# 0411tony/Yue

Hardware: AMD Instinct MI355X
Metric: BPR triplet-updates/sec at k=128 (S-round semantics, user rows sequential; the reference's exact sequential semantics: secondary.exact) (higher is better)
Workload: dtype f32

## Files before the change

### yue_amd/csrc/bpr_host.hip

```cpp
#include "host_common.hpp"

#include "train_kernels.hpp"
#include "round_kernels.hpp"

using yue_host::fail;
using yue_host::kr_of;
using yue_host::with_kr;
static_assert(yue::kNllSlots == yue_host::kNllSlotsHost && yue::kHeaderSlack == yue_host::kHeaderSlackHost &&
              yue::kMetaStageMax == (uint32_t)yue_host::kMetaStageMaxHost, "host_common.hpp mirrors these");

namespace {

yue::TrainArgs make_args(yue_ctx *c, double lr, double regU, double regI) {
    yue::TrainArgs a{};
    a.P = c->P.p; a.Q = c->Q.p; a.dP = c->dP.p; a.dQ = c->dQ.p;
    a.stage = c->Q.p ? c->Q.p + (size_t)c->n * c->k : nullptr;
    a.ev_u = c->ev_u.p; a.ev_i = c->ev_i.p; a.ev_j = c->ev_j.p;
    a.indptr = c->indptr.p; a.indices = c->indices.p;
    a.nll_slots = c->scal.p;
    a.m = c->m; a.n = c->n; a.k = c->k;
    a.lr = lr;
    a.ru = (float)(lr * regU);
    a.ri = (float)(lr * regI);
    a.neg_lo = 0; a.neg_range = (int32_t)c->n;
// ... 19 lines not shown
template <class F>
bool with_round_instance(int kr, int tpw, F &&f) {
    return with_round_instance(kr, tpw, f, std::make_index_sequence<sizeof kRoundInstances / sizeof kRoundInstances[0]>{});
}

int tpw_of(const yue_ctx *c, bool meta) { return c->opt_round_tpw ? c->opt_round_tpw : default_round_tpw(kr_of(c->k), meta); }

constexpr int64_t kMetaRangeMax = 37 * 1024;
constexpr int64_t kMetaRangesMax = 12;
constexpr int64_t kRoundGenerationsMax = 6;
constexpr double kRoundEventsPerItemRow = 4.0;

bool meta_bucketed(const yue_ctx *c) { return c->n > kMetaRangeMax * kMetaRangesMax || c->opt_round_bucket; }
bool meta_path_fits(const yue_ctx *c) { return c->opt_round_meta && c->n <= ((int64_t)yue::kBucketRangesMax << yue::kBucketShift); }

int default_round_events(yue_ctx *c, double n_rows, int64_t *out) {
    const bool fold = yue_host::fold_path(c);
    const int tpw = tpw_of(c, fold);
    int per_cu = 0, cus = 0;
    hipError_t e = hipSuccess;
    if (!with_round_instance(kr_of(c->k), tpw, [&](auto kr, auto t) {
            e = fold ? hipOccupancyMaxActiveBlocksPerMultiprocessor(&per_cu, yue::k_round_m<kr(), t()>, 256, 0)
                     : hipOccupancyMaxActiveBlocksPerMultiprocessor(&per_cu, yue::k_round<kr(), t()>, 256, 0);
        }))
        return fail(YUE_ERR_ARG, "unsupported (k, TPW) combination");
    HIPCHK(e);
    per_cu = std::min(per_cu, fold ? 7 : 6);
    HIPCHK(hipDeviceGetAttribute(&cus, hipDeviceAttributeMultiprocessorCount, c->device));
    const double slots = (double)per_cu * (double)cus;
    int64_t w = (int64_t)(slots * 4.0 * tpw);
    w -= w % 1024;
    w = std::max<int64_t>(w, 1024);
    if (fold) {
        int64_t sets = std::min<int64_t>(kRoundGenerationsMax, std::max<int64_t>(1, (int64_t)(kRoundEventsPerItemRow * n_rows / (double)w)));
        if (2.0 * (double)(w * sets) < 2.0 * n_rows) sets = std::min<int64_t>(sets, 4);
        w *= sets;
    }
    *out = w;
    return YUE_OK;
}

int launch_round(yue_ctx *c, const yue::TrainArgs &a_in, int64_t e0, int64_t e1, int64_t n0, int64_t n1,
                 int parity, int apply_p) {
    unsigned long long *cnt[2] = {c->cnt0.p, c->cnt1.p};
    uint32_t *cntp[2] = {c->cntp0.p, c->cntp1.p};
    yue::RoundArgs ra{};
    ra.e_begin = e0; ra.e_end = e1; ra.n_begin = n0; ra.n_end = n1;
    ra.cnt_cur = cnt[parity]; ra.cnt_next = cnt[parity ^ 1]; ra.cntp_cur = cntp[parity]; ra.cntp_next = cntp[parity ^ 1];
    uint32_t *tab[2] = {c->tab0.p, c->tab1.p};
    ra.tab_cur = tab[parity]; ra.tab_next = tab[parity ^ 1]; ra.staged = c->staged ? 1 : 0;
    ra.apply_p = apply_p;
    const int tpw = tpw_of(c, false);
    const int64_t waves = (std::max(e1 - e0, n1 - n0) + tpw - 1) / tpw;
    const int64_t blocks = (waves + 3) / 4;
    if (blocks == 0) return YUE_OK;
    const dim3 grid((unsigned)blocks), block(256);
#ifdef YUE_STAMPS
    yue::TrainArgs a = a_in;
    a.stamps = nullptr;
    if (e1 > e0 && c->update_launches++ == c->stamp_launch) {
        HIPCHK(c->stamps.resize((size_t)waves * 8));
        HIPCHK(hipMemsetAsync(c->stamps.p, 0, (size_t)waves * 64, c->stream));
        a.stamps = c->stamps.p;
        c->stamp_waves = (e1 - e0 + tpw - 1) / tpw;
    }
#else
    const yue::TrainArgs &a = a_in;
#endif
    if (!with_round_instance(kr_of(c->k), tpw, [&](auto kr, auto t) {
            hipLaunchKernelGGL((yue::k_round<kr(), t()>), grid, block, 0, c->stream, a, ra, a.ev_u, a.ev_i, a.ev_j);
        }))
        return fail(YUE_ERR_ARG, "unsupported (k, TPW) combination");
    return YUE_OK;
}

int launch_round_meta(yue_ctx *c, const yue::TrainArgs &a, const std::vector<int64_t> &bounds) {
    const int64_t R = (int64_t)bounds.size() - 1;
    const int64_t E = bounds.back();
    HIPCHK(c->meta_i.resize((size_t)E + yue::kHeaderSlack)); HIPCHK(c->meta_j.resize((size_t)E + yue::kHeaderSlack));
    HIPCHK(c->round_rows.resize((size_t)R)); HIPCHK(c->d_bounds.resize((size_t)R + 1));
    if (c->h_bounds != bounds) {
        HIPCHK(hipStreamSynchronize(c->stream));
        c->h_bounds = bounds;
        HIPCHK(hipMemcpyAsync(c->d_bounds.p, c->h_bounds.data(), (size_t)(R + 1) * sizeof(int64_t), hipMemcpyHostToDevice, c->stream));
    }
    HIPCHK(hipMemsetAsync(c->round_rows.p, 0, (size_t)R * sizeof(unsigned long long), c->stream));
    HIPCHK(c->fold.resize((size_t)(E + 4 * R + 8)));
    yue::MetaArgs ma{};
    ma.ev_i = a.ev_i; ma.ev_j = a.ev_j; ma.bounds = c->d_bounds.p; ma.R = R; ma.n = (int32_t)c->n;
    const bool bucketed = meta_bucketed(c);
    if (bucketed) {
        ma.range = 1 << yue::kBucketShift;
        ma.G = (int32_t)((c->n + ma.range - 1) >> yue::kBucketShift);
        HIPCHK(c->bk_touch.resize((size_t)(2 * E + 2))); HIPCHK(c->bk_ptr.resize((size_t)R * (ma.G + 1)));
        yue::BucketArgs ba{};
        ba.ev_i = a.ev_i; ba.ev_j = a.ev_j; ba.bounds = c->d_bounds.p; ba.R = R; ba.G = ma.G;
        ba.bk_touch = c->bk_touch.p; ba.bk_ptr = c->bk_ptr.p; ba.meta_i = c->meta_i.p; ba.meta_j = c->meta_j.p;
        int cus0 = 0;
        HIPCHK(hipDeviceGetAttribute(&cus0, hipDeviceAttributeMultiprocessorCount, c->device));
        hipLaunchKernelGGL(yue::k_round_bucket, dim3((unsigned)std::min<int64_t>(R, 2 * cus0)), dim3(1024), 0, c->stream, ba);
        ma.bk_touch = c->bk_touch.p; ma.bk_ptr = c->bk_ptr.p;
    } else {
        ma.G = (int32_t)((c->n + kMetaRangeMax - 1) / kMetaRangeMax);
        ma.range = (int32_t)((c->n + ma.G - 1) / ma.G);
    }
    ma.chunk = (ma.range + 1023) / 1024; ma.chunk |= 1;
    int64_t widest = 0;
    for (int64_t r = 0; r < R; ++r) widest = std::max(widest, bounds[(size_t)r + 1] - bounds[(size_t)r]);
    const double mean_touches = 2.0 * (double)widest / (double)std::max<int64_t>(1, c->n);
    const uint32_t stage_auto = (uint32_t)std::min<double>((double)yue::kMetaStageMax, std::max<double>((double)yue::kMetaStageDefault,
                                                         std::ceil(mean_touches * (kr_of(c->k) == 1 ? 4.0 : 2.0))));
    ma.stage_max = !c->staged ? 1u : c->opt_round_stage >= 2 ? (uint32_t)c->opt_round_stage : stage_auto;
    c->last_stage_max = (int)ma.stage_max;
    ma.meta_i = c->meta_i.p; ma.meta_j = c->meta_j.p; ma.round_rows = c->round_rows.p; ma.fold = c->fold.p;
    const size_t lds = (size_t)ma.range * sizeof(uint32_t);
    const void *kfn = bucketed ? (const void *)yue::k_round_meta<true> : (const void *)yue::k_round_meta<false>;
    HIPCHK(hipFuncSetAttribute(kfn, hipFuncAttributeMaxDynamicSharedMemorySize, (int)lds));
    int per_cu = 0, cus = 0;
    if (bucketed) { HIPCHK(hipOccupancyMaxActiveBlocksPerMultiprocessor(&per_cu, yue::k_round_meta<true>, 1024, lds)); }
    else { HIPCHK(hipOccupancyMaxActiveBlocksPerMultiprocessor(&per_cu, yue::k_round_meta<false>, 1024, lds)); }
    HIPCHK(hipDeviceGetAttribute(&cus, hipDeviceAttributeMultiprocessorCount, c->device));
    const int64_t grid = std::max<int64_t>(8, std::min<int64_t>((R * ma.G + 7) / 8 * 8, (int64_t)std::max(per_cu, 1) * cus / 8 * 8));
    if (bucketed) hipLaunchKernelGGL(yue::k_round_meta<true>, dim3((unsigned)grid), dim3(1024), lds, c->stream, ma);
    else
        hipLaunchKernelGGL(yue::k_round_meta<false>, dim3((unsigned)grid), dim3(1024), lds, c->stream, ma);
    HIPCHK(hipGetLastError());
    return YUE_OK;
}

void launch_round_fold(yue_ctx *c, const yue::TrainArgs &a, int64_t e0, int64_t e1, int64_t round_index) {
    yue::FoldArgs f{};
    f.fold = c->fold.p + yue::fold_base(e0, round_index); f.round_rows = c->round_rows.p + round_index; f.Q = a.Q; f.dQ = a.dQ; f.stage = a.stage; f.k = c->k; f.capacity = (uint32_t)((e1 - e0) & ~(int64_t)3);
    const dim3 fgrid((unsigned)std::min<int64_t>(c->opt_fold_blocks, std::max<int64_t>(1, (e1 - e0 + 15) / 16))), block(256);
    with_kr(c->k, [&](auto kr) { hipLaunchKernelGGL(yue::k_round_fold<kr()>, fgrid, block, 0, c->stream, f); });
}

int launch_round_m(yue_ctx *c, const yue::TrainArgs &a_in, int64_t e0, int64_t e1, int64_t round_index) {
    yue::RoundMArgs ra{};
    ra.e_begin = e0; ra.e_end = e1; ra.staged = c->staged ? 1 : 0;
    const int tpw = tpw_of(c, true);
    const int64_t waves = (e1 - e0 + tpw - 1) / tpw;
    const int64_t blocks = (waves + 3) / 4;
    if (blocks == 0) return YUE_OK;
    const dim3 grid((unsigned)blocks), block(256);
#ifdef YUE_STAMPS
    yue::TrainArgs a = a_in;
    a.stamps = nullptr;
    if (c->update_launches++ == c->stamp_launch) {
        HIPCHK(c->stamps.resize((size_t)waves * 8));
        HIPCHK(hipMemsetAsync(c->stamps.p, 0, (size_t)waves * 64, c->stream));
        a.stamps = c->stamps.p;
        c->stamp_waves = waves;
    }
#else
    const yue::TrainArgs &a = a_in;
#endif
    const uint32_t *mi = c->meta_i.p, *mj = c->meta_j.p;
    if (c->bigq) {
        bool is_default = false;
        with_round_instance(kr_of(c->k), tpw, [&](auto kr, auto t) {
            if constexpr (t() == default_round_tpw(kr(), true)) {
                hipLaunchKernelGGL((yue::k_round_m<kr(), t(), true>), grid, block, 0, c->stream, a, ra, a.ev_u, a.ev_i, a.ev_j, mi, mj);
                is_default = true;
            }
        });
        if (!is_default) return fail(YUE_ERR_ARG, "item matrices of 2 GiB and more: only the default events-per-wave setting (round_tpw = 0)");
    } else if (!with_round_instance(kr_of(c->k), tpw, [&](auto kr, auto t) {
                   hipLaunchKernelGGL((yue::k_round_m<kr(), t()>), grid, block, 0, c->stream, a, ra, a.ev_u, a.ev_i, a.ev_j, mi, mj);
               }))
        return fail(YUE_ERR_ARG, "unsupported (k, TPW) combination");
    launch_round_fold(c, a, e0, e1, round_index);
    return YUE_OK;
}

int launch_round_u(yue_ctx *c, const yue::TrainArgs &a, int64_t u0, int64_t u1, int64_t e0, int64_t e1, int64_t round_index) {
    yue::RoundUArgs ra{};
    ra.u_begin = u0; ra.u_end = u1; ra.ev_ptr = c->d_ev_ptr.p; ra.e_begin = e0; ra.e_end = e1; ra.staged = c->staged ? 1 : 0; ra.margins = c->margins.p;
    ra.psq_slots = c->psq_in_rounds ? c->psq_slots.p : nullptr;
    const int64_t blocks = (u1 - u0 + 3) / 4;
    if (blocks == 0) return YUE_OK;
    const dim3 grid((unsigned)blocks), block(256);
    const uint32_t *mi = c->meta_i.p, *mj = c->meta_j.p;
    with_kr(c->k, [&](auto kr) {
        if (c->opt_round_fast) hipLaunchKernelGGL((yue::k_round_u<kr(), true>), grid, block, 0, c->stream, a, ra, a.ev_i, a.ev_j, mi, mj);
        else hipLaunchKernelGGL((yue::k_round_u<kr(), false>), grid, block, 0, c->stream, a, ra, a.ev_i, a.ev_j, mi, mj);
    });
    launch_round_fold(c, a, e0, e1, round_index);
    return YUE_OK;
}

template <typename F>
int run_rounds(yue_ctx *c, yue::TrainArgs a, const std::vector<int64_t> &bounds, int apply_p, F after_round, bool meta = false, const std::vector<int64_t> *user_blocks = nullptr) {
    const int64_t R = (int64_t)bounds.size() - 1;
    int64_t widest = 0;
    for (int64_t r = 0; r < R; ++r) widest = std::max(widest, bounds[(size_t)r + 1] - bounds[(size_t)r]);
    if (widest >= (1ll << 24)) meta = false;
    const bool fits31 = (c->n + 2 * widest) * (int64_t)c->k * 4 < (1ll << 31);
    c->bigq = meta && !fits31;
    if (!meta && (int64_t)c->n * c->k * 4 >= (1ll << 31))
        return fail(YUE_ERR_ARG, "item matrices of 2 GiB and more per GPU are supported by yue_bpr_epoch's default path only (not by explicit rounds / round_meta = 0 / rounds of 2^24 events and more)");
    c->staged = c->opt_round_stage && widest > 0 && (fits31 || c->bigq);
    if (c->staged) {
        const size_t need = (size_t)(c->n + 2 * widest) * (size_t)c->k;
        if (c->Q.n < need) {
            DevBuf<float> bigger;
            HIPCHK(bigger.resize(need));
// ... 450 lines not shown
```

### yue_amd/csrc/core_host.hip

```cpp
#include "host_common.hpp"

namespace yue_host {
thread_local std::string g_err;
int fail(int code, const std::string &msg) { g_err = msg; return code; }
}
using yue_host::fail;
void yue_comm_release(yue_ctx *c);

extern "C" {

const char *yue_last_error(void) { return yue_host::g_err.c_str(); }
int yue_version(void) { return 1; }

int yue_ctx_create(int device, yue_ctx **out) {
    if (!out) return fail(YUE_ERR_ARG, "yue_ctx_create: out is NULL");
    int ndev = 0;
    HIPCHK(hipGetDeviceCount(&ndev));
    if (ndev <= 0) return fail(YUE_ERR_HIP, "no HIP device visible: libyue_hip needs an MI355X (no CPU fallback exists)");
    if (device < 0 || device >= ndev) return fail(YUE_ERR_ARG, "device ordinal out of range");
    HIPCHK(hipSetDevice(device));
    yue_ctx *c = new yue_ctx();
    c->device = device;
    const auto init = [c]() -> int {
        HIPCHK(hipStreamCreateWithFlags(&c->stream, hipStreamNonBlocking));
// ... 15 lines not shown

int yue_ctx_destroy(yue_ctx *c) {
    if (!c) return YUE_OK;
    (void)hipSetDevice(c->device);
    if (c->stream) (void)hipStreamSynchronize(c->stream);
    if (c->comm_stream) (void)hipStreamSynchronize(c->comm_stream);
    yue_comm_release(c);
    if (c->comm_stream) (void)hipStreamDestroy(c->comm_stream);
    if (c->stream) (void)hipStreamDestroy(c->stream);
    delete c;
    return YUE_OK;
}

int yue_sync(yue_ctx *c) {
    if (!c) return fail(YUE_ERR_ARG, "null context");
    HIPCHK(hipSetDevice(c->device));
    HIPCHK(hipStreamSynchronize(c->stream));
    return YUE_OK;
}

int yue_set_factors(yue_ctx *c, const float *P, int64_t m, const float *Q, int64_t n, int k) {
    if (!c || !P || !Q) return fail(YUE_ERR_ARG, "yue_set_factors: null argument");
    if (m <= 0 || n <= 0 || k <= 0 || k > 256) return fail(YUE_ERR_ARG, "yue_set_factors: need m,n > 0 and 1 <= k <= 256");
    if (n >= (1ll << 31) || m >= (1ll << 31)) return fail(YUE_ERR_ARG, "yue_set_factors: ids must fit int32");
    HIPCHK(hipSetDevice(c->device));
    if (c->have_inter && (m != c->m || n != c->n || k != c->k)) c->have_inter = false;
    if (k != c->k) c->opt_round_tpw = 0;
    c->m = m; c->n = n; c->k = k;
    HIPCHK(c->P.resize(m * k)); HIPCHK(c->Q.resize(n * k));
    HIPCHK(c->dP.resize(m * k)); HIPCHK(c->dQ.resize(n * k));
    HIPCHK(c->cnt0.resize(n)); HIPCHK(c->cnt1.resize(n)); HIPCHK(c->cntp0.resize(m)); HIPCHK(c->cntp1.resize(m));
    HIPCHK(hipMemcpyAsync(c->P.p, P, m * k * sizeof(float), hipMemcpyHostToDevice, c->stream));
    HIPCHK(hipMemcpyAsync(c->Q.p, Q, n * k * sizeof(float), hipMemcpyHostToDevice, c->stream));
    HIPCHK(hipMemsetAsync(c->dP.p, 0, m * k * sizeof(float), c->stream));
    HIPCHK(hipMemsetAsync(c->dQ.p, 0, n * k * sizeof(float), c->stream));
    HIPCHK(hipMemsetAsync(c->cntp0.p, 0, m * sizeof(uint32_t), c->stream));
    HIPCHK(hipMemsetAsync(c->cntp1.p, 0, m * sizeof(uint32_t), c->stream));
    HIPCHK(hipMemsetAsync(c->cnt0.p, 0, n * sizeof(unsigned long long), c->stream));
    HIPCHK(hipMemsetAsync(c->cnt1.p, 0, n * sizeof(unsigned long long), c->stream));
    HIPCHK(hipStreamSynchronize(c->stream));
    c->have_factors = true;
    return YUE_OK;
}

int yue_get_factors(yue_ctx *c, float *P, float *Q) {
    if (!c || !c->have_factors) return fail(YUE_ERR_ARG, "yue_get_factors: no factors uploaded");
    HIPCHK(hipSetDevice(c->device));
    if (P) HIPCHK(hipMemcpyAsync(P, c->P.p, c->m * c->k * sizeof(float), hipMemcpyDeviceToHost, c->stream));
    if (Q) HIPCHK(hipMemcpyAsync(Q, c->Q.p, c->n * c->k * sizeof(float), hipMemcpyDeviceToHost, c->stream));
    HIPCHK(hipStreamSynchronize(c->stream));
    return YUE_OK;
}

int yue_set_interactions(yue_ctx *c, const int64_t *indptr, const int32_t *indices, const int64_t *ev_ptr, const int32_t *ev_i) {
    if (!c || !indptr || !indices || !ev_ptr || !ev_i) return fail(YUE_ERR_ARG, "yue_set_interactions: null argument");
    if (!c->have_factors) return fail(YUE_ERR_ARG, "yue_set_interactions: call yue_set_factors first (m, n)");
    HIPCHK(hipSetDevice(c->device));
    const int64_t m = c->m, n = c->n;
    int rc = check_rows("yue_set_interactions: interaction", indptr, m, indices, n, yue_host::kNoTotal, Order::ascending);
    if (!rc) rc = check_rows("yue_set_interactions: event", ev_ptr, m, ev_i, n, yue_host::kNoTotal, Order::any);
    if (rc) return rc;
    for (int64_t u = 0; u < m; ++u)
        if (indptr[u + 1] - indptr[u] >= n) return fail(YUE_ERR_ARG, "yue_set_interactions: a user listened to every item (the reference's sampler would never return, BPR.py:47)");
    const int64_t nnz = indptr[m], E = ev_ptr[m];
    {
        int64_t prev = -1, max_gap = 0;
        for (int64_t u = 0; u < m; ++u) if (ev_ptr[u + 1] > ev_ptr[u]) { if (prev >= 0) max_gap = std::max(max_gap, u - prev); prev = u; }
        if (max_gap * c->k * 4 >= (1ll << 31)) return fail(YUE_ERR_ARG, "yue_set_interactions: more than 2 GiB of user-factor rows between two consecutive users with events");
    }
    std::vector<int32_t> evu((size_t)E);
    for (int64_t u = 0; u < m; ++u)
        for (int64_t e = ev_ptr[u]; e < ev_ptr[u + 1]; ++e) evu[(size_t)e] = (int32_t)u;
    c->E = E; c->nnz = nnz;
    c->h_ev_ptr.assign(ev_ptr, ev_ptr + m + 1);
    c->all_users_have_events = true;
    for (int64_t u = 0; u < m; ++u) if (ev_ptr[u + 1] <= ev_ptr[u]) { c->all_users_have_events = false; break; }
    c->d_ev_ptr_valid = false;
    HIPCHK(c->indptr.resize(m + 1)); HIPCHK(c->indices.resize(std::max<int64_t>(nnz, 1)));
    HIPCHK(c->ev_u.resize((size_t)E + yue_host::kHeaderSlackHost)); HIPCHK(c->ev_i.resize((size_t)E + yue_host::kHeaderSlackHost)); HIPCHK(c->ev_j.resize((size_t)E + yue_host::kHeaderSlackHost));
    HIPCHK(hipMemcpyAsync(c->indptr.p, indptr, (m + 1) * sizeof(int64_t), hipMemcpyHostToDevice, c->stream));
    HIPCHK(hipMemcpyAsync(c->indices.p, indices, nnz * sizeof(int32_t), hipMemcpyHostToDevice, c->stream));
    HIPCHK(hipMemcpyAsync(c->ev_u.p, evu.data(), E * sizeof(int32_t), hipMemcpyHostToDevice, c->stream));
    HIPCHK(hipMemcpyAsync(c->ev_i.p, ev_i, E * sizeof(int32_t), hipMemcpyHostToDevice, c->stream));
    HIPCHK(hipStreamSynchronize(c->stream));
    c->have_inter = true;
    return YUE_OK;
}


}
```

### yue_amd/csrc/host_common.hpp

```cpp
#pragma once
#include "../../include/yue_hip.h"
#include "input_checks.hpp"

#include <hip/hip_runtime.h>

#include <algorithm>
#include <cmath>
#include <cstdio>
#include <cstdlib>
#include <cstring>
#include <memory>
#include <string>
#include <type_traits>
#include <utility>
#include <vector>

struct ncclComm;
struct yue_wrmf;
struct yue_knn;
struct yue_expo;
struct yue_cof;
struct yue_cnet;
struct yue_s2v;
struct yue_lgcn;
// ... 49 lines not shown
    return YUE_OK;
}

struct Event {
    hipEvent_t e = nullptr;
    Event() = default;
    Event(const Event &) = delete;
    Event &operator=(const Event &) = delete;
    Event(Event &&o) noexcept : e(o.e) { o.e = nullptr; }
    Event &operator=(Event &&o) noexcept { std::swap(e, o.e); return *this; }
    ~Event() { if (e) (void)hipEventDestroy(e); }
    hipError_t create(unsigned flags = hipEventDefault) { return e ? hipSuccess : hipEventCreateWithFlags(&e, flags); }
    hipError_t record(hipStream_t s) {
        const hipError_t rc = create();
        return rc != hipSuccess ? rc : hipEventRecord(e, s);
    }
    operator hipEvent_t() const { return e; }
};

inline hipError_t elapsed(hipEvent_t from, hipEvent_t to, double *ms) {
    float f = 0.0f;
    const hipError_t rc = hipEventElapsedTime(&f, from, to);
    if (rc == hipSuccess) *ms = (double)f;
    return rc;
}
inline int64_t ns_of(double ms) { return (int64_t)(1e6 * ms); }
inline hipError_t elapsed(hipEvent_t from, hipEvent_t to, int64_t *ns) {
    double ms = 0.0;
    const hipError_t rc = elapsed(from, to, &ms);
    if (rc == hipSuccess) *ns = ns_of(ms);
    return rc;
}

constexpr int kNllSlotsHost = 1024;
constexpr int kHeaderSlackHost = 16;
constexpr int kMetaStageMaxHost = 64;
constexpr int kWrmfStageHost = 32;
constexpr int kKnnRangeHost = 4096, kKnnMaxKHost = 256, kKnnGatherHost = 2048;
constexpr int kCofRangeHost = 8192;

template <class T>
using StatePtr = std::unique_ptr<T, void (*)(T *)>;

inline int kr_of(int k) { return k <= 64 ? 1 : k <= 128 ? 2 : 4; }

template <class F>
auto with_kr(int k, F &&f) {
    switch (kr_of(k)) {
        case 1: return f(std::integral_constant<int, 1>{});
        case 2: return f(std::integral_constant<int, 2>{});
        default: return f(std::integral_constant<int, 4>{});
    }
}

}

using yue_host::DevBuf;
using yue_host::Event;
using yue_host::Order;
using yue_host::check_ids;
using yue_host::check_rows;
using yue_host::check_transpose;

struct yue_ctx {
    int device = 0;
    hipStream_t stream = nullptr;
    int64_t m = 0, n = 0, E = 0, nnz = 0;
    int k = 0;
    bool have_factors = false, have_inter = false;
    DevBuf<float> P, Q, dP, dQ;
    DevBuf<float> margins;
    DevBuf<double> psq_slots;
    DevBuf<unsigned long long> cnt0, cnt1;
    DevBuf<uint32_t> cntp0, cntp1;
    DevBuf<uint32_t> tab0, tab1;
    bool staged = false;
    bool bigq = false;
    DevBuf<uint32_t> meta_i, meta_j;
    DevBuf<unsigned long long> round_rows;
    DevBuf<uint2> fold, bk_touch;
    DevBuf<uint32_t> bk_ptr;
    DevBuf<int64_t> d_bounds;
    std::vector<int64_t> h_bounds;
#ifdef YUE_STAMPS
    DevBuf<unsigned long long> stamps;
    int64_t stamp_launch = -1, update_launches = 0, stamp_waves = 0;
#endif
    DevBuf<int32_t> ev_u, ev_i, ev_j, indices;
    DevBuf<int64_t> indptr;
    DevBuf<int32_t> xu, xi, xj, xk;
    DevBuf<double> x_loss;
    DevBuf<float> aU_m, aU_v, aV_m, aV_v;
    int64_t adam_m = 0, adam_n = 0; int adam_k = 0;
    DevBuf<double> scal;
    std::vector<int64_t> h_ev_ptr;
    bool all_users_have_events = false;
    bool psq_in_rounds = false;
    DevBuf<int32_t> s_users, s_ids, s_mask_idx, s_flags;
    DevBuf<int32_t> s_few, s_few_ids;
    DevBuf<float> s_few_scores;
    int64_t scan_few_users = 0;
    DevBuf<int64_t> s_mask_ptr;
    DevBuf<float> s_scores, s_row, s_norms;
    double scan_ms = 0.0;
    int64_t scan_events = 0, scan_rescored = 0, scan_tiles_done = 0, scan_tiles_total = 0;
    DevBuf<unsigned long long> s_work;
    DevBuf<unsigned short> s_qb;
    DevBuf<uint32_t> s_masks;
    int opt_scan_two_phase = 1;
    int64_t opt_scan_streams_min_users = 262144;
    int opt_scan_slabs = 4;
    int opt_scan_streams = 2;
    int opt_scan_filter_ub = 3;
    int opt_scan_growth = 0;
    int scan_chunks = 0;
    int scan_used_bf16 = 0;
    int opt_scan_f32 = 0;
    int opt_scan_batch = 0;
    int opt_round_tpw = 0;
    int opt_topn_true = 0;
    int scan_settle = 0;
    int last_stage_max = 0;
    int opt_round_stage = 1;
    int opt_round_bucket = 0;
    int opt_fold_blocks = 1536;
    int opt_round_user_seq = 1;
    int opt_round_fast = 1;
    int last_round_user_seq = 0;
    int opt_comm_group_mb = 8;
    int opt_round_cus_reserved = 0;
    int64_t comm_compute_waits = 0;
    int opt_round_meta = 1;
    int timing_stride = 0;
    std::vector<std::pair<Event, Event>> ev_pool;
    std::vector<int64_t> ev_triplets, ev_launches;
    size_t ev_used = 0;
    DevBuf<double> fP, fBi, f_coef, f_x, f_hist, f_scores, f_out_sc;
    DevBuf<float> fQ;
    DevBuf<int64_t> f_ptr;
    DevBuf<int32_t> f_items, f_negs, f_ids, f_flags;
    DevBuf<int64_t> f_uq_ptr, f_neg_ptr;
    DevBuf<int32_t> f_uq_items, f_loc_i, f_loc_j;
    DevBuf<float> f_wq, f_dQ;
    DevBuf<double> f_wp, f_wb, f_dP, f_dB;
    DevBuf<unsigned> f_cnt;
    int64_t fn = 0;
    int fk = 0;
    int opt_fism_inplace = 1;
    int opt_fism_lds = 1;
    int64_t fism_form = 0;
    DevBuf<uint32_t> ch_key, ch_val, ch_key2, ch_val2, ch_seg, ch_ord_i, ch_ord_j, ch_head, ch_incl, ch_ord_u, ch_rkey, ch_rval;
    DevBuf<int64_t> ch_run_ptr, d_ev_ptr;
    DevBuf<int32_t> ch_run_u;
    DevBuf<unsigned char> ch_tmp;
    DevBuf<unsigned> ch_Qv, ch_Pv;
    DevBuf<unsigned long long> ch_ctl;
    DevBuf<unsigned long long> ch_stats;
    bool d_ev_ptr_valid = false;
    int opt_epoch_exact = 0;
    int opt_replay_levels = 0;
    int opt_chain_split = -1;
    int opt_chain_ring = 0;
    int opt_chain_xcd = 0;
    int opt_chain_fast = 0;
    int opt_chain_waves = 0;
    int64_t opt_chain_spin = 0;
// ... 90 lines not shown
```

### yue_amd/csrc/options_host.hip

```cpp
#include "host_common.hpp"

#include <limits>

using yue_host::fail;

namespace {

struct Option {
    const char *name;
    int64_t (*get)(yue_ctx *);
    void (*put)(yue_ctx *, int64_t);
    int (*set)(const Option &, yue_ctx *, int64_t);
    int64_t lo, hi;
    const char *refusal;
    std::vector<int64_t> also;
};
#define YUE_AT(member) [](yue_ctx *c) -> int64_t { return c->member; }, [](yue_ctx *c, int64_t v) { c->member = (decltype(c->member))v; }
#define YUE_FROM(reader) [](yue_ctx *c) -> int64_t { return yue_host::reader; }

int set_flag(const Option &o, yue_ctx *c, int64_t value) { o.put(c, value != 0); return YUE_OK; }

int set_ranged(const Option &o, yue_ctx *c, int64_t value) {
    if ((value < o.lo || value > o.hi) && std::find(o.also.begin(), o.also.end(), value) == o.also.end())
        return fail(YUE_ERR_ARG, std::string("yue_set_option: ") + o.name + " " + o.refusal);
    o.put(c, value);
    return YUE_OK;
}

int64_t round_path(yue_ctx *c) { return yue_host::fold_path(c) ? 1 : 0; }

int set_round_cus_reserved(const Option &, yue_ctx *c, int64_t value) {
    int cus = 0;
    HIPCHK(hipSetDevice(c->device));
    HIPCHK(hipDeviceGetAttribute(&cus, hipDeviceAttributeMultiprocessorCount, c->device));
    if (value < 0 || value >= cus) return fail(YUE_ERR_ARG, "yue_set_option: round_cus_reserved must be 0 .. CUs - 1");
    HIPCHK(hipStreamSynchronize(c->stream));
    hipStream_t fresh = nullptr;
    if (value == 0) HIPCHK(hipStreamCreateWithFlags(&fresh, hipStreamNonBlocking));
    else {
        std::vector<uint32_t> mask((size_t)(cus + 31) / 32, 0u);
        for (int cu = 0; cu < cus - (int)value; ++cu) mask[(size_t)cu / 32] |= 1u << (cu % 32);
        HIPCHK(hipExtStreamCreateWithCUMask(&fresh, (uint32_t)mask.size(), mask.data()));
    }
    (void)hipStreamDestroy(c->stream);
    c->stream = fresh;
    c->opt_round_cus_reserved = (int)value;
    return YUE_OK;
}

int set_round_tpw(const Option &, yue_ctx *c, int64_t value) {
    if (value != 0 && value != 2 && value != 4 && value != 8 && value != 16) return fail(YUE_ERR_ARG, "yue_set_option: round_tpw must be 0, 2, 4, 8 or 16");
    if (value == 8 && yue_host::kr_of(c->k) == 4) return fail(YUE_ERR_ARG, "yue_set_option: round_tpw 8 needs k <= 128");
    if (value == 16 && yue_host::kr_of(c->k) != 1) return fail(YUE_ERR_ARG, "yue_set_option: round_tpw 16 needs k <= 64");
    c->opt_round_tpw = (int)value;
    return YUE_OK;
}

#ifdef YUE_STAMPS
int set_stamp_launch(const Option &, yue_ctx *c, int64_t value) { c->stamp_launch = value; c->update_launches = 0; return YUE_OK; }
#endif

constexpr int64_t kNoEnd = std::numeric_limits<int64_t>::max();

const Option kOptions[] = {
    {"scan_f32", YUE_AT(opt_scan_f32), set_flag},
    {"scan_batch", YUE_AT(opt_scan_batch), set_ranged, 0, 1, "must be 0 or 1"},
    {"scan_two_phase", YUE_AT(opt_scan_two_phase), set_flag},
    {"scan_growth", YUE_AT(opt_scan_growth), set_ranged, 2, 64, "must be 0 (automatic) or 2..64", {0}},
    {"scan_filter_ub", YUE_AT(opt_scan_filter_ub), set_ranged, 1, 3, "must be 1, 2 or 3"},
    {"scan_streams", YUE_AT(opt_scan_streams), set_ranged, 1, 2, "must be 1 or 2"},
    {"scan_slabs", YUE_AT(opt_scan_slabs), set_ranged, 2, 64, "must be 2..64"},
    {"scan_streams_min_users", YUE_AT(opt_scan_streams_min_users), set_ranged, 1024, kNoEnd, "must be at least 1024"},
    {"scan_last_chunks", YUE_AT(scan_chunks)},
    {"scan_last_few_users", YUE_AT(scan_few_users)},
    {"scan_last_settle", YUE_AT(scan_settle)},
    {"topn_true", YUE_AT(opt_topn_true), set_flag},
    {"fism_lds", YUE_AT(opt_fism_lds), set_flag},
    {"fism_inplace", YUE_AT(opt_fism_inplace), set_flag},
    {"fism_last_form", YUE_AT(fism_form)},
    {"round_stage", YUE_AT(opt_round_stage), set_ranged, 0, yue_host::kMetaStageMaxHost, "must be 0, 1 or 2..64"},
    {"round_last_stage_max", YUE_AT(last_stage_max)},
    {"round_meta", YUE_AT(opt_round_meta), set_flag},
    {"comm_group_mb", YUE_AT(opt_comm_group_mb), set_ranged, 1, 4096, "must be 1..4096"},
    {"round_cus_reserved", YUE_AT(opt_round_cus_reserved), set_round_cus_reserved},
    {"comm_last_compute_waits", YUE_AT(comm_compute_waits)},
    {"round_user_seq", YUE_AT(opt_round_user_seq), set_flag},
    {"round_fast", YUE_AT(opt_round_fast), set_flag},
    {"round_last_user_seq", YUE_AT(last_round_user_seq)},
    {"round_bucket", YUE_AT(opt_round_bucket), set_flag},
    {"fold_blocks", YUE_AT(opt_fold_blocks), set_ranged, 1, 65536, "out of range"},
    {"round_tpw", YUE_AT(opt_round_tpw), set_round_tpw},
    {"round_path", round_path},
#ifdef YUE_STAMPS
    {"debug_stamp_launch", nullptr, nullptr, set_stamp_launch},
#endif
    {"epoch_exact", YUE_AT(opt_epoch_exact), set_flag},
    {"replay_levels", YUE_AT(opt_replay_levels), set_flag},
    {"chain_waves", YUE_AT(opt_chain_waves), set_ranged, 0, 8, "must be 0..8"},
    {"chain_split", YUE_AT(opt_chain_split), set_ranged, -1, 1, "must be -1, 0 or 1"},
    {"chain_fast", YUE_AT(opt_chain_fast), set_flag},
    {"chain_xcd", YUE_AT(opt_chain_xcd), set_flag},
    {"chain_ring", YUE_AT(opt_chain_ring), set_ranged, 0, 0, "must be 0, 8 or 16", {8, 16}},
    {"chain_spin", YUE_AT(opt_chain_spin), set_ranged, 0, 0x7fffffff, "out of range"},
    {"chain_last_us", YUE_AT(chain_kernel_us)},
    {"chain_last_runs", YUE_AT(chain_runs)},
    {"chain_last_waves", YUE_AT(chain_waves)},
    {"replay_last_levels", YUE_AT(replay_levels)},
    {"lgcn_hub", YUE_AT(opt_lgcn_hub), set_ranged, 1, 0x7fffffff, "must be 1 .. 2^31 - 1"},
    {"lgcn_last_hubs", YUE_AT(lgcn_hubs)},
    {"lgcn_last_parts", YUE_AT(lgcn_parts)},
    {"lgcn_last_forward_ns", YUE_AT(lgcn_ns[0])},
    {"lgcn_last_batch_ns", YUE_AT(lgcn_ns[1])},
    {"lgcn_last_backward_ns", YUE_AT(lgcn_ns[2])},
    {"lgcn_last_adam_ns", YUE_AT(lgcn_ns[3])},
    {"ngcf_hub", YUE_AT(opt_ngcf_hub), set_ranged, 1, 0x7fffffff, "must be 1 .. 2^31 - 1"},
    {"ngcf_last_hubs", YUE_AT(ngcf_hubs)},
    {"ngcf_last_parts", YUE_AT(ngcf_parts)},
    {"ngcf_last_gather_ns", YUE_AT(ngcf_ns[0])},
    {"ngcf_last_dense_ns", YUE_AT(ngcf_ns[1])},
    {"ngcf_last_batch_ns", YUE_AT(ngcf_ns[2])},
    {"ngcf_last_backward_ns", YUE_AT(ngcf_ns[3])},
    {"ngcf_last_wgrad_ns", YUE_AT(ngcf_ns[4])},
    {"ngcf_last_adam_ns", YUE_AT(ngcf_ns[5])},
    {"cdae_hub", YUE_AT(opt_cdae_hub), set_ranged, 1, 0x7fffffff, "must be 1 .. 2^31 - 1"},
    {"cdae_last_hubs", YUE_AT(cdae_hubs)},
    {"cdae_last_parts", YUE_AT(cdae_parts)},
    {"cdae_last_saturated", YUE_AT(cdae_saturated)},
    {"apr_last_longest_row", YUE_AT(apr_longest)},
    {"wrmf_long_pairs", YUE_AT(opt_wrmf_long_pairs), set_ranged, yue_host::kWrmfStageHost, kNoEnd, "must be >= 32"},
    {"wrmf_last_ns", YUE_AT(wrmf_ns[0])},
    {"wrmf_last_long_ns", YUE_AT(wrmf_ns[1])},
    {"wrmf_long_rows_user", YUE_FROM(wrmf_long_rows(c, 0))},
    {"wrmf_long_rows_item", YUE_FROM(wrmf_long_rows(c, 1))},
    {"knn_range", YUE_AT(opt_knn_range), set_ranged, 64, yue_host::kKnnRangeHost, "must be 64..4096"},
    {"knn_gather", YUE_AT(opt_knn_gather), set_ranged, yue_host::kKnnMaxKHost, yue_host::kKnnGatherHost, "must be 256..2048"},
    {"knn_last_ns", YUE_AT(knn_ns)},
    {"knn_last_chunked_users", YUE_AT(knn_chunked_users)},
    {"ipf_slots", YUE_AT(opt_ipf_slots), set_ranged, 1, 4096, "must be 1..4096"},
    {"ipf_last_ns", YUE_AT(ipf_ns)},
    {"expo_gram_mb", YUE_AT(opt_expo_gram_mb), set_ranged, 1, 65536, "must be in [1, 65536]"},
    {"expo_last_ns", YUE_AT(expo_ns[0])},
    {"expo_last_gram_ns", YUE_AT(expo_ns[1])},
    {"expo_last_batches", YUE_AT(expo_batches)},
    {"cof_cooccur_mb", YUE_AT(opt_cof_cooccur_mb), set_ranged, 1, 65536, "must be in [1, 65536]"},
    {"cof_level_timing", YUE_AT(opt_cof_level_timing), set_ranged, 0, 1, "must be 0 or 1"},
    {"cof_pass_items", YUE_AT(opt_cof_pass_items), set_ranged, 64, yue_host::kCofRangeHost, "must be in [64, 8192]"},
    {"cof_last_ns", YUE_AT(cof_ns[0])},
    {"cof_last_small_ns", YUE_AT(cof_ns[1])},
    {"cof_levels", YUE_FROM(cof_levels(c))},
    {"cof_cooccur_nnz", YUE_FROM(cof_cooccur_nnz(c))},
    {"cnet_last_ns", YUE_AT(cnet_ns)},
    {"s2v_schedule", YUE_AT(opt_s2v_schedule), set_ranged, 0, 1, "must be 0 (one wave walks all steps) or 1 (levels)"},
    {"s2v_levels_steps", YUE_FROM(s2v_levels(c, 0))},
    {"s2v_levels_pairs", YUE_FROM(s2v_levels(c, 1))},
    {"s2v_last_ns", YUE_AT(s2v_ns)},
};
#undef YUE_AT
#undef YUE_FROM

const Option *find_option(const std::string &key) {
    for (const Option &o : kOptions) if (key == o.name) return &o;
    return nullptr;
}

}

extern "C" {

int yue_get_option(yue_ctx *c, const char *name, int64_t *value) {
    if (!c || !name || !value) return fail(YUE_ERR_ARG, "yue_get_option: null argument");
    const std::string key(name);
    const Option *o = find_option(key);
    if (o && o->get) { *value = o->get(c); return YUE_OK; }
    return fail(YUE_ERR_ARG, "yue_get_option: unknown option " + key);
}
// ... 11 lines not shown
```

### yue_amd/csrc/round_kernels.hpp

```cpp
#pragma once
#include "train_kernels.hpp"

#ifdef YUE_ABL_NO_HOT
#define YUE_M_HOT(val, rs, vo, so) asm volatile("" :: "v"(val))
#else
#define YUE_M_HOT(val, rs, vo, so) YUE_BATOMIC(val, rs, vo, so)
#endif
#ifdef YUE_ABL_NO_DP
#define YUE_M_DP(val, rs, vo, so) asm volatile("" :: "v"(val))
#else
#define YUE_M_DP(val, rs, vo, so) YUE_BATOMIC(val, rs, vo, so)
#endif

#define YUE_BLOAD_NT(rs, vo, so) __builtin_bit_cast(float, __builtin_amdgcn_raw_buffer_load_b32((rs), (vo), (so), 2))
#if defined(YUE_EXP_LOAD_CACHED)
#define YUE_M_LOAD_J(rs, vo, so) YUE_BLOAD(rs, vo, so)
#define YUE_M_LOAD_I(rs, vo, so) YUE_BLOAD(rs, vo, so)
#elif defined(YUE_EXP_LOAD_NT)
#define YUE_M_LOAD_J(rs, vo, so) YUE_BLOAD_NT(rs, vo, so)
#define YUE_M_LOAD_I(rs, vo, so) YUE_BLOAD_NT(rs, vo, so)
#else
#define YUE_M_LOAD_J(rs, vo, so) YUE_BLOAD_NT(rs, vo, so)
#define YUE_M_LOAD_I(rs, vo, so) YUE_BLOAD(rs, vo, so)
#endif

#define YUE_FOLD_LD(p) __builtin_nontemporal_load(p)
#define YUE_FOLD_LDROW(p) (*(p))

namespace yue {

constexpr uint32_t kMetaStageMax = 64u;
constexpr uint32_t kMetaStageDefault = 4u;
constexpr uint32_t kMetaUnique = 1u, kMetaStaged = 2u, kMetaHot = 3u;
constexpr uint32_t kMetaFirst = 1u << 31;
constexpr int kMetaUnroll = 8;
__host__ __device__ inline uint32_t meta_kind(uint32_t w) { return w & 3u; }
__host__ __device__ inline uint32_t meta_slot(uint32_t w) { return (w >> 2) & 0x1fffffffu; }
__host__ __device__ inline bool meta_first(uint32_t w) { return (w & kMetaFirst) != 0u; }
__host__ __device__ inline uint32_t fold_count(uint32_t w) { return w >> 25; }
__host__ __device__ inline uint32_t fold_block(uint32_t w) { return w & 0x1ffffffu; }
constexpr uint32_t kLdsStaged = 1u << 31, kLdsTicket = 1u << 25;
static_assert(kMetaStageMax <= 64u, "tickets of a block must fit bits 25..30 of the LDS word");
__device__ inline uint32_t meta_of_staged(uint32_t lds) {
    const uint32_t ticket = (lds >> 25) & 63u;
    return kMetaStaged | (((lds & 0x1ffffffu) + ticket) << 2) | (ticket == 0u ? kMetaFirst : 0u);
}

struct MetaArgs {
    const int32_t *ev_i, *ev_j;
    const int64_t *bounds;
    int64_t R;
    int32_t n;
    int32_t range;
    int32_t G;
    int32_t chunk;
    uint32_t stage_max;
    uint32_t *meta_i, *meta_j;
    unsigned long long *round_rows;
    uint2 *fold;
    const uint2 *bk_touch;
    const uint32_t *bk_ptr;
};

__host__ __device__ inline int64_t fold_base(int64_t e0, int64_t r) { return (e0 + 4 * r + 3) & ~(int64_t)3; }

template <bool BUCKETED>
__global__ void __launch_bounds__(1024) k_round_meta(MetaArgs a) {
    extern __shared__ uint32_t slots[];
    __shared__ unsigned long long wsum[16];
    __shared__ unsigned long long range_base;
    const int tid = threadIdx.x, lane = tid & 63, wv = tid >> 6;
    const int64_t xcd = blockIdx.x & 7, local = blockIdx.x >> 3, per_xcd = gridDim.x >> 3;
    const int64_t rounds_here = (a.R - xcd + 7) >> 3;
    for (int64_t sq = local; sq < rounds_here * a.G; sq += per_xcd) {
        const int64_t r = (sq / a.G) * 8 + xcd;
        const int32_t g = (int32_t)(sq % a.G);
        const int32_t lo = g * a.range;
        const int32_t width = min(a.range, a.n - lo);
        const int64_t e0 = a.bounds[r], e1 = a.bounds[r + 1];
        for (int s = tid; s < a.range; s += 1024) slots[s] = 0u;
        __syncthreads();
        const uint2 *mine_t = nullptr;
        uint32_t mine_n = 0u;
        if (BUCKETED) {
            const uint32_t *bp = a.bk_ptr + r * (a.G + 1) + g;
            mine_t = a.bk_touch + 2 * e0 + bp[0];
            mine_n = bp[1] - bp[0];
        }
        if (BUCKETED) {
            for (uint32_t t = tid; t < mine_n; t += 1024) atomicAdd(&slots[mine_t[t].x - (uint32_t)lo], 1u);
        } else {
        for (int64_t eb = e0 + tid; eb < e1; eb += 1024 * kMetaUnroll) {
            int32_t vi[kMetaUnroll], vj[kMetaUnroll];
#pragma unroll
            for (int q = 0; q < kMetaUnroll; ++q) {
                const int64_t e = eb + 1024 * q;
                vj[q] = e < e1 ? a.ev_j[e] : -1; vi[q] = e < e1 ? a.ev_i[e] : 0;
            }
#pragma unroll
            for (int q = 0; q < kMetaUnroll; ++q)
                if (vj[q] >= 0) {
                    const uint32_t si = (uint32_t)(vi[q] - lo), sj = (uint32_t)(vj[q] - lo);
                    if (si < (uint32_t)width) atomicAdd(&slots[si], 1u);
                    if (sj < (uint32_t)width) atomicAdd(&slots[sj], 1u);
                }
        }
        }
        __syncthreads();
        const int s0 = tid * a.chunk;
        unsigned long long mine = 0ull;
        for (int q = 0; q < a.chunk; ++q) {
            const int s = s0 + q;
            if (s < width) { const uint32_t c = slots[s]; if (c >= 2u) mine += (1ull << 32) + (c <= a.stage_max ? c : 0u); }
        }
        unsigned long long incl = mine;
#pragma unroll
        for (int off = 1; off < 64; off <<= 1) { const unsigned long long up = __shfl_up(incl, off); if (lane >= off) incl += up; }
        if (lane == 63) wsum[wv] = incl;
        __syncthreads();
        if (tid == 0) {
            unsigned long long total = 0ull;
            for (int q = 0; q < 16; ++q) total += wsum[q];
            range_base = total ? atomicAdd(a.round_rows + r, total) : 0ull;
        }
        __syncthreads();
        unsigned long long run = range_base + incl - mine;
        for (int q = 0; q < wv; ++q) run += wsum[q];
        uint2 *fold = a.fold + fold_base(e0, r);
        for (int q = 0; q < a.chunk; ++q) {
            const int s = s0 + q;
            if (s < width) {
                const uint32_t c = slots[s];
                if (c >= 2u) {
                    const bool st = c <= a.stage_max;
                    slots[s] = st ? (kLdsStaged | ((uint32_t)run & 0x1ffffffu)) : kMetaHot;
                    fold[run >> 32] = make_uint2((uint32_t)(lo + s), st ? ((c << 25) | ((uint32_t)run & 0x1ffffffu)) : 0u);
                    run += (1ull << 32) + (st ? c : 0u);
                }
            }
        }
        __syncthreads();
        if (BUCKETED) {
            for (uint32_t t = tid; t < mine_n; t += 1024) {
                const uint2 tc = mine_t[t];
                const uint32_t sl = tc.x - (uint32_t)lo;
                const uint32_t wd = slots[sl];
                const uint32_t mw = (wd & kLdsStaged) ? meta_of_staged(atomicAdd(&slots[sl], kLdsTicket)) : wd;
                ((tc.y & 1u) ? a.meta_j : a.meta_i)[e0 + (tc.y >> 1)] = mw;
            }
        } else
        for (int64_t eb = e0 + tid; eb < e1; eb += 1024 * kMetaUnroll) {
            int32_t vi[kMetaUnroll], vj[kMetaUnroll];
#pragma unroll
            for (int q = 0; q < kMetaUnroll; ++q) {
                const int64_t e = eb + 1024 * q;
                vj[q] = e < e1 ? a.ev_j[e] : -1; vi[q] = e < e1 ? a.ev_i[e] : 0;
            }
#pragma unroll
            for (int q = 0; q < kMetaUnroll; ++q) {
                const int64_t e = eb + 1024 * q;
                if (vj[q] >= 0) {
                    const uint32_t si = (uint32_t)(vi[q] - lo), sj = (uint32_t)(vj[q] - lo);
                    if (si < (uint32_t)width) {
                        const uint32_t wd = slots[si];
                        a.meta_i[e] = (wd & kLdsStaged) ? meta_of_staged(atomicAdd(&slots[si], kLdsTicket)) : wd;
                    }
                    if (sj < (uint32_t)width) {
                        const uint32_t wd = slots[sj];
                        a.meta_j[e] = (wd & kLdsStaged) ? meta_of_staged(atomicAdd(&slots[sj], kLdsTicket)) : wd;
                    }
                } else if (g == 0 && e < e1) {
                    a.meta_i[e] = 0u; a.meta_j[e] = 0u;
                }
            }
        }
        __syncthreads();
    }
}

constexpr int kBucketShift = 15;
constexpr int kBucketRangesMax = 256;
struct BucketArgs {
    const int32_t *ev_i, *ev_j;
    const int64_t *bounds;
    int64_t R;
    int32_t G;
    uint2 *bk_touch;
    uint32_t *bk_ptr;
    uint32_t *meta_i, *meta_j;
};

__global__ void __launch_bounds__(1024) k_round_bucket(BucketArgs a) {
    __shared__ uint32_t cnt[kBucketRangesMax], off[kBucketRangesMax + 1];
    const int tid = threadIdx.x;
    for (int64_t r = blockIdx.x; r < a.R; r += gridDim.x) {
        const int64_t e0 = a.bounds[r], e1 = a.bounds[r + 1];
        for (int g = tid; g < a.G; g += 1024) cnt[g] = 0u;
        __syncthreads();
        for (int64_t eb = e0 + tid; eb < e1; eb += 1024 * kMetaUnroll) {
            int32_t vi[kMetaUnroll], vj[kMetaUnroll];
#pragma unroll
            for (int q = 0; q < kMetaUnroll; ++q) {
                const int64_t e = eb + 1024 * q;
                vj[q] = e < e1 ? a.ev_j[e] : 0; vi[q] = e < e1 ? a.ev_i[e] : -1;
            }
#pragma unroll
            for (int q = 0; q < kMetaUnroll; ++q) {
                if (vi[q] < 0) continue;
                if (vj[q] >= 0) { atomicAdd(&cnt[vi[q] >> kBucketShift], 1u); atomicAdd(&cnt[vj[q] >> kBucketShift], 1u); }
                else { a.meta_i[eb + 1024 * q] = 0u; a.meta_j[eb + 1024 * q] = 0u; }
            }
        }
        __syncthreads();
        if (tid == 0) {
            uint32_t run = 0u;
            for (int g = 0; g < a.G; ++g) { off[g] = run; run += cnt[g]; cnt[g] = 0u; }
            off[a.G] = run;
        }
        __syncthreads();
        for (int g = tid; g <= a.G; g += 1024) a.bk_ptr[r * (a.G + 1) + g] = off[g];
        uint2 *dst = a.bk_touch + 2 * e0;
        for (int64_t eb = e0 + tid; eb < e1; eb += 1024 * kMetaUnroll) {
            int32_t vi[kMetaUnroll], vj[kMetaUnroll];
#pragma unroll
            for (int q = 0; q < kMetaUnroll; ++q) {
                const int64_t e = eb + 1024 * q;
                vj[q] = e < e1 ? a.ev_j[e] : -1; vi[q] = e < e1 ? a.ev_i[e] : 0;
            }
#pragma unroll
            for (int q = 0; q < kMetaUnroll; ++q)
                if (vj[q] >= 0) {
                    const uint32_t code = 2u * (uint32_t)(eb + 1024 * q - e0);
                    const int gi = vi[q] >> kBucketShift, gj = vj[q] >> kBucketShift;
                    dst[off[gi] + atomicAdd(&cnt[gi], 1u)] = make_uint2((uint32_t)vi[q], code);
                    dst[off[gj] + atomicAdd(&cnt[gj], 1u)] = make_uint2((uint32_t)vj[q], code | 1u);
                }
        }
        __syncthreads();
    }
}


struct RoundMArgs {
    int64_t e_begin, e_end;
    int staged;
};

template <int KR, int TPW, bool BIGQ = false>
__global__ void __launch_bounds__(256) __attribute__((amdgpu_num_sgpr(96))) k_round_m(TrainArgs a, RoundMArgs ra, const int32_t *__restrict__ evu,
                                                 const int32_t *__restrict__ evi, const int32_t *__restrict__ evj,
                                                 const uint32_t *__restrict__ mti, const uint32_t *__restrict__ mtj) {
    const int lane = threadIdx.x & 63;
    const int64_t wave = (int64_t)blockIdx.x * 4 + __builtin_amdgcn_readfirstlane((int)(threadIdx.x >> 6));
    const int64_t base = ra.e_begin + wave * TPW;
    if (base >= ra.e_end) return;
    YUE_STAMP(0, "");

// ... 399 lines not shown
```

Baseline: 1.785 billion.

## Cache per-round positive-item touch counts across epochs in meta pre-pass

Adds a one-time kernel that counts positive-item touches per round and range and packs them as saturating 8-bit counts. The meta kernel then seeds its LDS histogram from this cache and only atomically adds negative-item touches. This drops half the per-epoch ev_i reads and LDS atomics. The cost is extra device memory, a cold-path correction for invalid events, a saturation bias encoding and cache invalidation logic.

Result: no change. 1.787 billion (median of 6 runs) (+0.1%).

```diff
diff --git a/yue_amd/csrc/bpr_host.hip b/yue_amd/csrc/bpr_host.hip
--- a/yue_amd/csrc/bpr_host.hip
+++ b/yue_amd/csrc/bpr_host.hip
@@ -125,6 +125,7 @@
     if (c->h_bounds != bounds) {
         HIPCHK(hipStreamSynchronize(c->stream));
         c->h_bounds = bounds;
+        c->pos_cnt_valid = false;
         HIPCHK(hipMemcpyAsync(c->d_bounds.p, c->h_bounds.data(), (size_t)(R + 1) * sizeof(int64_t), hipMemcpyHostToDevice, c->stream));
     }
     HIPCHK(hipMemsetAsync(c->round_rows.p, 0, (size_t)R * sizeof(unsigned long long), c->stream));
@@ -156,15 +157,31 @@
     ma.stage_max = !c->staged ? 1u : c->opt_round_stage >= 2 ? (uint32_t)c->opt_round_stage : stage_auto;
     c->last_stage_max = (int)ma.stage_max;
     ma.meta_i = c->meta_i.p; ma.meta_j = c->meta_j.p; ma.round_rows = c->round_rows.p; ma.fold = c->fold.p;
-    const size_t lds = (size_t)ma.range * sizeof(uint32_t);
-    const void *kfn = bucketed ? (const void *)yue::k_round_meta<true> : (const void *)yue::k_round_meta<false>;
+    ma.pos_words = (ma.range + 3) / 4;
+    const int64_t pos_total = R * ma.G * (int64_t)ma.pos_words;
+    const bool static_pos = !bucketed && c->opt_meta_static_pos && a.ev_i == c->ev_i.p && pos_total * 4 <= (c->opt_meta_static_cap_mb << 20);
+    c->last_meta_static = static_pos ? 1 : 0;
+    const size_t lds = (size_t)(static_pos ? 4 * ma.pos_words : ma.range) * sizeof(uint32_t);
+    const void *kfn = bucketed ? (const void *)yue::k_round_meta<true> : static_pos ? (const void *)yue::k_round_meta<false, true> : (const void *)yue::k_round_meta<false>;
     HIPCHK(hipFuncSetAttribute(kfn, hipFuncAttributeMaxDynamicSharedMemorySize, (int)lds));
     int per_cu = 0, cus = 0;
     if (bucketed) { HIPCHK(hipOccupancyMaxActiveBlocksPerMultiprocessor(&per_cu, yue::k_round_meta<true>, 1024, lds)); }
+    else if (static_pos) { HIPCHK(hipOccupancyMaxActiveBlocksPerMultiprocessor(&per_cu, yue::k_round_meta<false, true>, 1024, lds)); }
     else { HIPCHK(hipOccupancyMaxActiveBlocksPerMultiprocessor(&per_cu, yue::k_round_meta<false>, 1024, lds)); }
     HIPCHK(hipDeviceGetAttribute(&cus, hipDeviceAttributeMultiprocessorCount, c->device));
+    if (static_pos && !(c->pos_cnt_valid && c->pos_range == ma.range && c->pos_G == ma.G)) {
+        HIPCHK(c->pos_cnt.resize((size_t)std::max<int64_t>(pos_total, 1)));
+        HIPCHK(hipFuncSetAttribute((const void *)yue::k_round_pos, hipFuncAttributeMaxDynamicSharedMemorySize, (int)lds));
+        const int64_t pgrid = std::max<int64_t>(1, std::min<int64_t>(R * ma.G, (int64_t)std::max(per_cu, 1) * cus));
+        hipLaunchKernelGGL(yue::k_round_pos, dim3((unsigned)pgrid), dim3(1024), lds, c->stream, ma, c->pos_cnt.p);
+        HIPCHK(hipGetLastError());
+        c->pos_cnt_valid = true; c->pos_range = ma.range; c->pos_G = ma.G;
+        c->pos_builds++;
+    }
+    ma.pos = static_pos ? c->pos_cnt.p : nullptr;
     const int64_t grid = std::max<int64_t>(8, std::min<int64_t>((R * ma.G + 7) / 8 * 8, (int64_t)std::max(per_cu, 1) * cus / 8 * 8));
     if (bucketed) hipLaunchKernelGGL(yue::k_round_meta<true>, dim3((unsigned)grid), dim3(1024), lds, c->stream, ma);
+    else if (static_pos) hipLaunchKernelGGL((yue::k_round_meta<false, true>), dim3((unsigned)grid), dim3(1024), lds, c->stream, ma);
     else
         hipLaunchKernelGGL(yue::k_round_meta<false>, dim3((unsigned)grid), dim3(1024), lds, c->stream, ma);
     HIPCHK(hipGetLastError());
diff --git a/yue_amd/csrc/core_host.hip b/yue_amd/csrc/core_host.hip
--- a/yue_amd/csrc/core_host.hip
+++ b/yue_amd/csrc/core_host.hip
@@ -121,6 +121,7 @@
     HIPCHK(hipMemcpyAsync(c->indices.p, indices, nnz * sizeof(int32_t), hipMemcpyHostToDevice, c->stream));
     HIPCHK(hipMemcpyAsync(c->ev_u.p, evu.data(), E * sizeof(int32_t), hipMemcpyHostToDevice, c->stream));
     HIPCHK(hipMemcpyAsync(c->ev_i.p, ev_i, E * sizeof(int32_t), hipMemcpyHostToDevice, c->stream));
+    c->pos_cnt_valid = false;
     HIPCHK(hipStreamSynchronize(c->stream));
     c->have_inter = true;
     return YUE_OK;
diff --git a/yue_amd/csrc/host_common.hpp b/yue_amd/csrc/host_common.hpp
--- a/yue_amd/csrc/host_common.hpp
+++ b/yue_amd/csrc/host_common.hpp
@@ -155,6 +155,13 @@
     DevBuf<uint32_t> bk_ptr;
     DevBuf<int64_t> d_bounds;
     std::vector<int64_t> h_bounds;
+    DevBuf<uint32_t> pos_cnt;
+    bool pos_cnt_valid = false;
+    int32_t pos_range = 0, pos_G = 0;
+    int64_t pos_builds = 0;
+    int last_meta_static = 0;
+    int opt_meta_static_pos = 1;
+    int64_t opt_meta_static_cap_mb = 256;
 #ifdef YUE_STAMPS
     DevBuf<unsigned long long> stamps;
     int64_t stamp_launch = -1, update_launches = 0, stamp_waves = 0;
diff --git a/yue_amd/csrc/options_host.hip b/yue_amd/csrc/options_host.hip
--- a/yue_amd/csrc/options_host.hip
+++ b/yue_amd/csrc/options_host.hip
@@ -91,6 +91,10 @@
     {"fold_blocks", YUE_AT(opt_fold_blocks), set_ranged, 1, 65536, "out of range"},
     {"round_tpw", YUE_AT(opt_round_tpw), set_round_tpw},
     {"round_path", round_path},
+    {"meta_static_pos", YUE_AT(opt_meta_static_pos), set_flag},
+    {"meta_static_cap_mb", YUE_AT(opt_meta_static_cap_mb), set_ranged, 0, 65536, "must be 0..65536"},
+    {"meta_static_builds", YUE_AT(pos_builds)},
+    {"meta_static_last", YUE_AT(last_meta_static)},
 #ifdef YUE_STAMPS
     {"debug_stamp_launch", nullptr, nullptr, set_stamp_launch},
 #endif
diff --git a/yue_amd/csrc/round_kernels.hpp b/yue_amd/csrc/round_kernels.hpp
--- a/yue_amd/csrc/round_kernels.hpp
+++ b/yue_amd/csrc/round_kernels.hpp
@@ -60,12 +60,17 @@
     uint2 *fold;
     const uint2 *bk_touch;
     const uint32_t *bk_ptr;
+    const uint32_t *pos;
+    int32_t pos_words;
 };
+constexpr uint32_t kPosSat = 255u, kPosSatBias = 1u << 26;
+constexpr int kPosUnroll = 10;
 
 __host__ __device__ inline int64_t fold_base(int64_t e0, int64_t r) { return (e0 + 4 * r + 3) & ~(int64_t)3; }
 
-template <bool BUCKETED>
+template <bool BUCKETED, bool STATIC_POS = false>
 __global__ void __launch_bounds__(1024) k_round_meta(MetaArgs a) {
+    static_assert(!(BUCKETED && STATIC_POS), "the bucketed pre-pass reads its own touch lists");
     extern __shared__ uint32_t slots[];
     __shared__ unsigned long long wsum[16];
     __shared__ unsigned long long range_base;
@@ -78,6 +83,24 @@
         const int32_t lo = g * a.range;
         const int32_t width = min(a.range, a.n - lo);
         const int64_t e0 = a.bounds[r], e1 = a.bounds[r + 1];
+        if (STATIC_POS) {
+            const uint32_t *pw = a.pos + (r * a.G + g) * (int64_t)a.pos_words;
+            for (int w0 = tid; w0 < a.pos_words; w0 += 1024 * kPosUnroll) {
+                uint32_t four[kPosUnroll];
+#pragma unroll
+                for (int q = 0; q < kPosUnroll; ++q) { const int w = w0 + 1024 * q; four[q] = w < a.pos_words ? pw[w] : 0u; }
+#pragma unroll
+                for (int q = 0; q < kPosUnroll; ++q) {
+                    const int w = w0 + 1024 * q;
+                    if (w < a.pos_words)
+#pragma unroll
+                        for (int b = 0; b < 4; ++b) {
+                            const uint32_t cnt = (four[q] >> (8 * b)) & 0xffu;
+                            slots[w + b * a.pos_words] = cnt == kPosSat ? kPosSat + kPosSatBias : cnt;
+                        }
+                }
+            }
+        } else
         for (int s = tid; s < a.range; s += 1024) slots[s] = 0u;
         __syncthreads();
         const uint2 *mine_t = nullptr;
@@ -89,6 +112,28 @@
         }
         if (BUCKETED) {
             for (uint32_t t = tid; t < mine_n; t += 1024) atomicAdd(&slots[mine_t[t].x - (uint32_t)lo], 1u);
+        } else if (STATIC_POS) {
+        bool gave_up = false;
+        for (int64_t eb = e0 + tid; eb < e1; eb += 1024 * kMetaUnroll) {
+            int32_t vj[kMetaUnroll];
+#pragma unroll
+            for (int q = 0; q < kMetaUnroll; ++q) {
+                const int64_t e = eb + 1024 * q;
+                vj[q] = e < e1 ? a.ev_j[e] : 0x7fffffff;
+            }
+#pragma unroll
+            for (int q = 0; q < kMetaUnroll; ++q) {
+                const uint32_t sj = (uint32_t)(vj[q] - lo);
+                if (vj[q] < 0) gave_up = true;
+                else if (sj < (uint32_t)width) atomicAdd(&slots[sj], 1u);
+            }
+        }
+        if (__syncthreads_or(gave_up))
+            for (int64_t e = e0 + tid; e < e1; e += 1024)
+                if (a.ev_j[e] < 0) {
+                    const uint32_t si = (uint32_t)(a.ev_i[e] - lo);
+                    if (si < (uint32_t)width) atomicSub(&slots[si], 1u);
+                }
         } else {
         for (int64_t eb = e0 + tid; eb < e1; eb += 1024 * kMetaUnroll) {
             int32_t vi[kMetaUnroll], vj[kMetaUnroll];
@@ -173,6 +218,38 @@
                     a.meta_i[e] = 0u; a.meta_j[e] = 0u;
                 }
             }
+        }
+        __syncthreads();
+    }
+}
+
+__global__ void __launch_bounds__(1024) k_round_pos(MetaArgs a, uint32_t *__restrict__ pos) {
+    extern __shared__ uint32_t slots[];
+    const int tid = threadIdx.x;
+    for (int64_t wi = blockIdx.x; wi < a.R * a.G; wi += gridDim.x) {
+        const int64_t r = wi / a.G;
+        const int32_t lo = (int32_t)(wi % a.G) * a.range;
+        const int32_t width = min(a.range, a.n - lo);
+        const int64_t e0 = a.bounds[r], e1 = a.bounds[r + 1];
+        for (int s = tid; s < 4 * a.pos_words; s += 1024) slots[s] = 0u;
+        __syncthreads();
+        for (int64_t eb = e0 + tid; eb < e1; eb += 1024 * kMetaUnroll) {
+            int32_t vi[kMetaUnroll];
+#pragma unroll
+            for (int q = 0; q < kMetaUnroll; ++q) { const int64_t e = eb + 1024 * q; vi[q] = e < e1 ? a.ev_i[e] : -1; }
+#pragma unroll
+            for (int q = 0; q < kMetaUnroll; ++q) {
+                const uint32_t si = (uint32_t)(vi[q] - lo);
+                if (vi[q] >= 0 && si < (uint32_t)width) atomicAdd(&slots[si], 1u);
+            }
+        }
+        __syncthreads();
+        uint32_t *pw = pos + wi * (int64_t)a.pos_words;
+        for (int w = tid; w < a.pos_words; w += 1024) {
+            uint32_t four = 0u;
+#pragma unroll
+            for (int b = 0; b < 4; ++b) four |= min(slots[w + b * a.pos_words], kPosSat) << (8 * b);
+            pw[w] = four;
         }
         __syncthreads();
     }
```
